# xflouris/libpll

Hardware: AMD Instinct MI355X
Metric: M CLV-site-updates/s (4x4 states x rates) (higher is better)
Workload: dtype f64

## Files before the change

### include/pll_amd.h

```cpp
#ifndef PLL_AMD_H_
#define PLL_AMD_H_

#include <stddef.h>
#include <stdint.h>
#include <stdio.h>

#ifdef __cplusplus
extern "C" {
#endif

#define PLL_EXPORT __attribute__((visibility("default")))


#define PLL_FAILURE 0
#define PLL_SUCCESS 1
#define PLL_FALSE 0
#define PLL_TRUE 1

#define PLL_ASCII_SIZE 256

#define PLL_SCALE_FACTOR 0x1p+256
#define PLL_SCALE_THRESHOLD 0x1p-256
#define PLL_SCALE_BUFFER_NONE (-1)
#define PLL_SCALE_RATE_MAXDIFF 4
// ... 885 lines not shown
PLL_EXPORT int pll_amd_set_deferral(pll_partition_t * partition, int on);
PLL_EXPORT int pll_amd_set_unstored_pairs(pll_partition_t * partition, int on);
PLL_EXPORT int pll_amd_unstored_stats(pll_partition_t * partition, unsigned long long * stats4);
PLL_EXPORT int pll_amd_set_pair_fold(pll_partition_t * partition, int on);
PLL_EXPORT int pll_amd_pair_fold_stats(pll_partition_t * partition, unsigned long long * stats4);
PLL_EXPORT int pll_amd_set_pair_row_capacity(pll_partition_t * partition, unsigned int rows);
PLL_EXPORT int pll_amd_pair_row_stats(pll_partition_t * partition, unsigned long long * stats4);
PLL_EXPORT int pll_amd_set_quad_rows(pll_partition_t * partition, int on, unsigned int min_sites_per_class);
PLL_EXPORT int pll_amd_set_quad_row_capacity(pll_partition_t * partition, unsigned int rows);
PLL_EXPORT int pll_amd_quad_row_stats(pll_partition_t * partition, unsigned long long * stats5);
PLL_EXPORT int pll_amd_quad_list_stats(pll_partition_t * partition, unsigned long long * stats3);
PLL_EXPORT int pll_amd_set_unstored_quad_products(pll_partition_t * partition, int on);
PLL_EXPORT int pll_amd_quad_product_stats(pll_partition_t * partition, unsigned long long * stats4);
PLL_EXPORT int pll_amd_set_quad_fold(pll_partition_t * partition, int on);
PLL_EXPORT int pll_amd_quad_fold_stats(pll_partition_t * partition, unsigned long long * stats4);
PLL_EXPORT int pll_amd_set_edge_fold(pll_partition_t * partition, int on);
PLL_EXPORT int pll_amd_edge_fold_stats(pll_partition_t * partition, unsigned long long * stats4);
PLL_EXPORT void * pll_amd_dev_clv(pll_partition_t * partition, unsigned int clv_index);

PLL_EXPORT int pll_amd_write_ceiling(pll_partition_t * partition, const pll_operation_t * operations, unsigned int count,
                                     unsigned int reps, float * ms_per_pass, double * bytes_per_pass);
PLL_EXPORT int pll_amd_list_kinds(pll_partition_t * partition, unsigned int * kinds8);
PLL_EXPORT int pll_amd_placement_info(pll_partition_t * partition, double * gbs, unsigned int cap, int * kept);
PLL_EXPORT int pll_amd_arena_fill_bandwidth(pll_partition_t * partition, double * gbs);

#ifdef __cplusplus
}
#endif
#endif
```

### include/pllhip.h

```cpp
#ifndef PLLHIP_H_
#define PLLHIP_H_

#include <stddef.h>
#include <stdint.h>

#ifdef __cplusplus
extern "C" {
#endif

#define PLLHIP_EXPORT __attribute__((visibility("default")))

typedef struct pllhip_ctx pllhip_ctx_t;

typedef struct pllhip_shape
{
  int device;
  unsigned int states;
  unsigned int rate_cats;
  unsigned int sites;
  unsigned int tips;
  unsigned int clv_buffers;
  unsigned int rate_matrices;
  unsigned int prob_matrices;
  unsigned int scale_buffers;
// ... 141 lines not shown
                                                      unsigned int lane);
PLLHIP_EXPORT int pllhip_fused_plan_dry_quads(unsigned int tips, unsigned int clv_buffers, unsigned int scale_buffers,
                                              int pattern_tip, unsigned int rate_cats, int rate_scalers, const pllhip_op_t * ops,
                                              unsigned int count, unsigned int nslots, const unsigned char * pinned,
                                              const int * edge4, unsigned int sites, int quads_on,
                                              unsigned int min_sites_per_class, const unsigned int * classes,
                                              const double * bounds, unsigned int * nkept, unsigned int * order_out,
                                              unsigned char * folded_out, int * ops_out, int * quads_out,
                                              unsigned int * counts_out);
PLLHIP_EXPORT int pllhip_fused_quad_rule_dry(int cherries, int instance, unsigned int n, unsigned int sites,
                                             unsigned int min_sites_per_class, int scales, double bound);
PLLHIP_EXPORT int pllhip_set_unstored_quad_products(pllhip_ctx_t * ctx, int on);
PLLHIP_EXPORT int pllhip_quad_product_stats(pllhip_ctx_t * ctx, unsigned long long * out4);
PLLHIP_EXPORT int pllhip_set_quad_fold(pllhip_ctx_t * ctx, int on);
PLLHIP_EXPORT int pllhip_quad_fold_stats(pllhip_ctx_t * ctx, unsigned long long * out4);
PLLHIP_EXPORT int pllhip_fused_plan_dry_quad_fold(unsigned int tips, unsigned int clv_buffers, unsigned int scale_buffers,
                                                  int pattern_tip, unsigned int rate_cats, int rate_scalers,
                                                  const pllhip_op_t * ops, unsigned int count, unsigned int nslots,
                                                  const unsigned char * pinned, const int * edge4, unsigned int sites,
                                                  int quads_on, unsigned int min_sites_per_class,
                                                  const unsigned int * classes, const double * bounds, int fold_on,
                                                  unsigned int * nkept, unsigned int * order_out, unsigned char * folded_out,
                                                  int * ops_out, int * quads_out, unsigned int * counts_out,
                                                  unsigned char * products_out, unsigned int * bytes_out,
                                                  unsigned char * qfolded_out, unsigned int * walked_out);
PLLHIP_EXPORT int pllhip_fused_plan_dry_quad_products(unsigned int tips, unsigned int clv_buffers, unsigned int scale_buffers,
                                                      int pattern_tip, unsigned int rate_cats, int rate_scalers,
                                                      const pllhip_op_t * ops, unsigned int count, unsigned int nslots,
                                                      const unsigned char * pinned, const int * edge4, unsigned int sites,
                                                      int quads_on, unsigned int min_sites_per_class,
// ... 305 lines not shown
```

### libpll_amd/csrc/hip/ctx.hip

```cpp
#include <dlfcn.h>
#include <sched.h>
#include <time.h>
#include <stdarg.h>
#include <stdlib.h>
#include <string.h>

#include <rccl/rccl.h>

#include <algorithm>
#include <string>
#include <vector>

#include <atomic>
#include "ctx.hpp"
#include "numerics.hpp"

static thread_local char g_err[512] = "";

void pllhip_set_error(const char * fmt, ...)
{
  va_list ap;
  va_start(ap, fmt);
  vsnprintf(g_err, sizeof(g_err), fmt, ap);
  va_end(ap);
// ... 298 lines not shown
    auto up = [](size_t b) { return (b + 4095) & ~(size_t)4095; };
    char * base = nullptr;
    if ((rc = alloc_arena_placed(c, &base, up(clv_b) + up(tip_b) + up(sc_b), shape->pattern_tip ? 0 : shape->tips,
                                 shape->clv_buffers, c->clv_stride * sizeof(double)))) goto fail;
    c->clv_arena = reinterpret_cast<double *>(base);
    if (tip_b) c->tipchars = reinterpret_cast<unsigned char *>(base + up(clv_b));
    c->scaler_arena = reinterpret_cast<unsigned int *>(base + up(clv_b) + up(tip_b));
    c->clv_arena_alloc_bytes = clv_b;
  }
  c->clv_arena_bytes = n_clv * c->clv_elems * sizeof(double);
  c->clv.assign(nodes, nullptr);
  for (unsigned int i = first; i < nodes; ++i)
    c->clv[i] = c->clv_arena + (size_t)(i - first) * c->clv_stride;
  if ((rc = dev_alloc(&c->pmatrix, (size_t)shape->prob_matrices * c->pmat_elems, true,
                      c->stream))) goto fail;
  if ((rc = dev_alloc(&c->eigenvals, (size_t)shape->rate_matrices * S, true, c->stream))) goto fail;
  if ((rc = dev_alloc(&c->eigenvecs, (size_t)shape->rate_matrices * S * S, true, c->stream))) goto fail;
  if ((rc = dev_alloc(&c->inv_eigenvecs, (size_t)shape->rate_matrices * S * S, true, c->stream))) goto fail;
  if ((rc = dev_alloc(&c->freqs, (size_t)shape->rate_matrices * S, true, c->stream))) goto fail;
  if ((rc = dev_alloc(&c->prop_invar, (size_t)shape->rate_matrices, true, c->stream))) goto fail;
  c->h_prop_invar.assign(shape->rate_matrices, 0.0);
  if ((rc = dev_alloc(&c->rates, R, true, c->stream))) goto fail;
  if ((rc = dev_alloc(&c->rate_weights, R, true, c->stream))) goto fail;
  if ((rc = dev_alloc(&c->pattern_weights, N + PLLHIP_TAIL_SITES, true, c->stream))) goto fail;
  if ((rc = dev_alloc(&c->tipmap, (size_t)256, true, c->stream))) goto fail;
  if ((rc = dev_alloc(&c->block_partials, (size_t)PLLHIP_REDUCE_BLOCKS * 2, true, c->stream))) goto fail;
  if ((rc = dev_alloc(&c->d_result, (size_t)4, true, c->stream))) goto fail;
  if ((rc = dev_alloc(&c->d_zero, (size_t)64, true, c->stream))) goto fail;
  HIP_TRY(hipHostMalloc((void **)&c->h_result, 4 * sizeof(double), hipHostMallocMapped));
  HIP_TRY(hipHostGetDevicePointer((void **)&c->h_result_dev, c->h_result, 0));
// ... 378 lines not shown
  if (!rc && freqs) rc = h2d(c, c->freqs + pi * S, freqs, S * sizeof(double));
  if (!rc) rc = h2d(c, c->prop_invar + pi, &prop_invar, sizeof(double));
  c->h_prop_invar[pi] = prop_invar;
  c->any_prop_invar = false;
  for (double p : c->h_prop_invar)
    if (p > 0) c->any_prop_invar = true;
  return rc;
}

extern "C" int pllhip_put_pmatrix(pllhip_ctx_t * c, unsigned int idx, const double * h)
{
  pllhip_edge_terms_drop(c);
  PLLHIP_ALL_SHARDS(c, pllhip_put_pmatrix(s, idx, h));
  PLLHIP_CERT_FIRST(c);
  if (idx >= c->sh.prob_matrices) { pllhip_set_error("pllhip_put_pmatrix: index %u", idx); return -1; }
  if (idx < c->pmat_min_entry.size() && c->pmat_min_entry[idx] != 0.0)
  {
    c->pmat_min_entry[idx] = c->pmat_min_rowsum[idx] = 0.0;
    ++c->layout_epoch;
  }
  return h2d(c, pllhip_pmat_ptr(c, idx), h, c->pmat_elems * sizeof(double));
}

extern "C" int pllhip_put_scaler(pllhip_ctx_t * c, unsigned int idx, const unsigned int * h)
{
  pllhip_edge_terms_drop(c);
  PLLHIP_ALL_SHARDS(c, pllhip_put_scaler(s, idx, h + lo * (c->sh.rate_scalers ? c->sh.rate_cats : 1)));
  PLLHIP_CERT_FIRST(c);
  if (idx >= c->sh.scale_buffers) { pllhip_set_error("pllhip_put_scaler: index %u", idx); return -1; }
  PLLHIP_DEFERRED_NEED(c, ~0u, ~0u, idx, -1);
// ... 376 lines not shown
```

### libpll_amd/csrc/hip/ctx.hpp

```cpp
#pragma once

#include <hip/hip_runtime.h>
#include <stdint.h>
#include <stdio.h>
#include <string.h>
#include <utility>
#include <vector>

#include "pllhip.h"

#define PLLHIP_MAX_RATE_CATS 64
#define PLLHIP_REDUCE_BLOCKS 65536
#define PLLHIP_HOSTSUM_MAX 8192

struct ncclComm;

struct pllhip_rep_work;

struct BatchScratch
{
  void * p = nullptr;
  size_t bytes = 0;
};
enum
// ... 16 lines not shown
  UNSTORED_NONE,
  UNSTORED_CHERRY,
  UNSTORED_PAIR,
  UNSTORED_FOLDED,
  UNSTORED_QUAD,
  UNSTORED_QUAD_FOLDED,
  UNSTORED_KINDS
};

struct pllhip_replicates
{
  pllhip_ctx * ctx;
  void * d_weights;
  size_t pitch;
  unsigned int count, width;
};

struct pllhip_ctx
{
  pllhip_shape_t sh;
  hipStream_t stream = nullptr;

  std::vector<pllhip_ctx *> shards;
  std::vector<size_t> shard_lo;
  bool shard_threads = true, shard_poll = true;
  bool shard_pin = false;
  struct pllhip_shard_pool * pool = nullptr;
  bool defer = false;
  unsigned long long pending_seq = 0;
  bool pending_hostsum = false, pending_spin = false, pending_stream_work = false;
// ... 74 lines not shown
    unsigned int * h_counts = nullptr;
    std::vector<quad_row> rows;
    unsigned int want = 0;
    unsigned int nstale = 0;
    unsigned long long clock = 0;
    unsigned long long stats[5] = {0, 0, 0, 0, 0};
  } quad_rows;
  bool quad_rows_on = true;
  unsigned int quad_min_sites_per_class = 64;
  std::vector<double> pmat_min_entry, pmat_min_rowsum;
  std::vector<double> h_eigenvals, h_eigenvecs, h_inv_eigenvecs, h_rates;
  std::vector<unsigned int> fused_last_quad_mats;
  unsigned int fused_last_quads_refused_by_bound = 0;
  unsigned int fused_last_quad_jobs = 0;
  unsigned long long quad_list_stats[3] = {0, 0, 0};
  struct deferred_clv
  {
    unsigned char kind = UNSTORED_NONE;
    unsigned int clv = 0;
    int scaler = -1;
    struct { unsigned int tip1 = 0, tip2 = 0; } cherry;
    struct { unsigned int rows[4] = {0, 0, 0, 0}; } pair;
    struct
    {
      unsigned int row[2] = {0, 0};
      unsigned int tips[2][4] = {{0, 0, 0, 0}, {0, 0, 0, 0}};
      unsigned int slot = 0;
    } quad;
    bool live() const { return kind != UNSTORED_NONE; }
    bool is_pair() const { return kind == UNSTORED_PAIR || kind == UNSTORED_FOLDED; }
// ... 233 lines not shown
static inline unsigned int * pllhip_scaler_ptr(const pllhip_ctx * c, int idx)
{
  return idx < 0 ? nullptr : c->scaler_arena + (size_t)idx * c->scaler_stride;
}

static inline const unsigned char * pllhip_tip_ptr(const pllhip_ctx * c, unsigned int tip)
{
  return c->tipchars + (size_t)tip * c->tip_stride;
}

static inline double * pllhip_pmat_ptr(const pllhip_ctx * c, unsigned int idx)
{
  return c->pmatrix + (size_t)idx * c->pmat_elems;
}

#define PLLHIP_INFINITY_CACHE_BYTES ((size_t)256 << 20)
static inline bool pllhip_use_nt(const pllhip_ctx * c)
{
  if (c->nt_override >= 0) return c->nt_override != 0;
  return c->clv_arena_bytes >= PLLHIP_INFINITY_CACHE_BYTES;
}

#define PLLHIP_STREAM_BLOCKS_PER_CU 256

static inline unsigned int pllhip_stream_grid(const pllhip_ctx * c, size_t items,
                                              unsigned int block)
{
  size_t need = (items + block - 1) / block;
  const size_t cap = (size_t)c->num_cus * PLLHIP_STREAM_BLOCKS_PER_CU;
  if (need < 1) need = 1;
// ... 135 lines not shown
```

### libpll_amd/csrc/hip/partials_fused.hip

```cpp
#include <algorithm>
#include <stdio.h>
#include <stdlib.h>
#include <type_traits>
#include <vector>

#include "ctx.hpp"
#include "numerics.hpp"
#include "partials_fused.hpp"

#define PLL_LDS __attribute__((address_space(3)))
#define PLL_GLOBAL __attribute__((address_space(1)))
typedef pll_v2d PLL_GLOBAL * global_v2d;
template <bool NT>
__device__ __forceinline__ void st16g(unsigned long long base, unsigned int byte_offset, double a, double b)
{
  const global_v2d p = (global_v2d)(base + byte_offset);
  const pll_v2d v = {a, b};
  if (NT) __builtin_nontemporal_store(v, p);
  else *p = v;
}

typedef const unsigned int __attribute__((address_space(4))) * const_words;
typedef const unsigned long long __attribute__((address_space(4))) * const_quads;
struct Rec
// ... 17 lines not shown
__device__ __forceinline__ unsigned int rec_req_rmat(const Rec & r) { return r.w[5]; }
__device__ __forceinline__ unsigned int rec_gather(const Rec & r) { return r.w[6]; }
__device__ __forceinline__ unsigned int rec_flags(const Rec & r) { return r.w[7]; }
__device__ __forceinline__ unsigned long long rec_parent(const Rec & r) { return rec_quad(r, 8); }
__device__ __forceinline__ unsigned long long rec_pscaler(const Rec & r) { return rec_quad(r, 10); }
__device__ __forceinline__ unsigned int rec_lslot(const Rec & r) { return r.w[12] & 0xffffu; }
__device__ __forceinline__ unsigned int rec_rslot(const Rec & r) { return r.w[12] >> 16; }
__device__ __forceinline__ unsigned int rec_pslot(const Rec & r) { return r.w[13] & 0xffffu; }
__device__ __forceinline__ unsigned int rec_src(const Rec & r) { return r.w[13] >> 16; }
__device__ __forceinline__ unsigned int rec_lcnt(const Rec & r) { return r.w[14] & 0xffffu; }
__device__ __forceinline__ unsigned int rec_rcnt(const Rec & r) { return r.w[14] >> 16; }
__device__ __forceinline__ unsigned int rec_pcnt(const Rec & r) { return r.w[15] & 0xffffu; }

constexpr unsigned int PLLHIP_QUAD_TABLE_WGS = 16;
template <int RC>
__global__ __launch_bounds__(256) void k_dna_quad_tables(const FusedPairJob * __restrict__ jobs, unsigned int njobs)
{
  const unsigned int i = blockIdx.x / PLLHIP_QUAD_TABLE_WGS, part = blockIdx.x % PLLHIP_QUAD_TABLE_WGS;
  if (i + 1 >= njobs || jobs[i].kind != 4) return;
  constexpr unsigned int ROW = RC * 4u, PER = 256u / ROW;
  const unsigned int ki = threadIdx.x % ROW, sub = threadIdx.x / ROW, rate4 = (ki >> 2) * 4u;
  const FusedPairJob & ja = jobs[i], & jb = jobs[i + 1];
  const PLL_GLOBAL double * pm = (const PLL_GLOBAL double *)ja.pmat;
  const PLL_GLOBAL unsigned short * patterns = (const PLL_GLOBAL unsigned short *)ja.kept;
  const unsigned int n = (unsigned int)ja.pad;
  const PLL_GLOBAL double * side_l[2] = {(const PLL_GLOBAL double *)ja.lmat, (const PLL_GLOBAL double *)jb.lmat};
  const PLL_GLOBAL double * side_r[2] = {(const PLL_GLOBAL double *)ja.rmat, (const PLL_GLOBAL double *)jb.rmat};
  const PLL_GLOBAL double * side_p[2] = {(const PLL_GLOBAL double *)jb.pmat, (const PLL_GLOBAL double *)jb.kept};
  const PLL_GLOBAL double * side_kept[2] = {(const PLL_GLOBAL double *)jb.copy, (const PLL_GLOBAL double *)jb.pad};
  double * tab = ja.tab;
  double * copy = ja.copy;
  double p[4], pf[2][4][4], l[2][4][4], r[2][4][4];
#pragma unroll
  for (int k = 0; k < 4; ++k) p[k] = pm[ki * 4u + k];
// ... 19 lines not shown
      double t[4];
#pragma unroll
      for (int k = 0; k < 4; ++k)
        t[k] = side_kept[s] ? side_kept[s][pair * ROW + rate4 + k] : masksum4(l[s][k], c1) * masksum4(r[s][k], c2);
#pragma unroll
      for (int k = 0; k < 4; ++k) f[s][k] = dot4(pf[s][k], t[0], t[1], t[2], t[3]);
    }
    const double q = dot4(p, f[0][0] * f[1][0], f[0][1] * f[1][1], f[0][2] * f[1][2], f[0][3] * f[1][3]);
    tab[cls * ROW + ki] = q;
    if (copy) copy[cls * ROW + ki] = q;
  }
}

template <int RC>
__global__ __launch_bounds__(256) void k_dna_pair_tables(const FusedPairJob * __restrict__ jobs, unsigned int njobs,
                                                         unsigned int * __restrict__ tile_counters)
{
  const unsigned int i = blockIdx.x >> 2, quarter = blockIdx.x & 3u;
  if (blockIdx.x == 0 && tile_counters) tile_counters[threadIdx.x * 32u] = 0u;
  if (i >= njobs) return;
  if (jobs[i].kind >= 4) return;
  if (jobs[i].kind >= 2)
  {
    constexpr unsigned int ROW = RC * 4u, PER = 256u / ROW, ROUNDS = 64u / PER;
    const unsigned int ki = threadIdx.x % ROW, sub = threadIdx.x / ROW, rate4 = (ki >> 2) * 4u;
    const PLL_GLOBAL double * pm = (const PLL_GLOBAL double *)jobs[i].pmat;
    double * tab = jobs[i].tab;
    double * copy = jobs[i].copy;
    double p[4];
#pragma unroll
    for (int k = 0; k < 4; ++k) p[k] = pm[ki * 4u + k];
    if (jobs[i].kind == 2)
    {
      const PLL_GLOBAL double * lm = (const PLL_GLOBAL double *)jobs[i].lmat, * rm = (const PLL_GLOBAL double *)jobs[i].rmat;
      double l[4][4], r[4][4];
// ... 1008 lines not shown
  if (f.rsc_slot >= 0) e.flags |= PLLHIP_FUSED_RCNT;
  e.lslot_b = (unsigned short)(f.lslot * in.slot.tile_bytes);
  e.rslot_b = (unsigned short)(f.rslot * in.slot.tile_bytes);
  e.lcnt_b = (unsigned short)((f.lsc_slot > 0 ? f.lsc_slot : 0) * in.slot.count_bytes);
  e.rcnt_b = (unsigned short)((f.rsc_slot > 0 ? f.rsc_slot : 0) * in.slot.count_bytes);
}

static void fused_encode(const FusedEncodeIn & in, const std::vector<std::vector<FusedOp>> & plans, const FusedAdmitted & adm,
                         const std::vector<FusedPairJob> * keep_jobs, const FusedEdge * edge, FusedEncoded & out)
{
  out.longest = adm.longest;
  for (size_t sg = 0; sg < plans.size(); ++sg) fused_encode_segment(in, plans[sg], adm.segs[sg], edge, out);
  if (keep_jobs) out.jobs.insert(out.jobs.end(), keep_jobs->begin(), keep_jobs->end());
}

static int fused_upload(pllhip_ctx * c, const FusedEncoded & enc)
{
  const size_t rec_bytes = enc.recs.size() * sizeof(FusedRec);
  const size_t seg_bytes = (size_t)PLLHIP_FUSED_MAX_SEGS * sizeof(FusedSeg);
  const size_t src_bytes = (enc.srcs.size() + 1) * sizeof(FusedSrc);
  const size_t job_bytes = (enc.jobs.size() + 1) * sizeof(FusedPairJob);
  const size_t tab_bytes = enc.rowtab.size() * sizeof(unsigned long long);
  const size_t segs_at = rec_bytes, srcs_at = segs_at + seg_bytes, jobs_at = srcs_at + src_bytes, rowtab_at = jobs_at + job_bytes;
  const size_t bytes = rowtab_at + tab_bytes;
  if (c->plan_cap < bytes)
  {
    HIP_TRY(hipStreamSynchronize(c->stream));
    for (int b = 0; b < 2; ++b)
    {
      if (c->h_plan[b]) HIP_TRY(hipHostFree(c->h_plan[b]));
// ... 13 lines not shown
  if (c->plan_pending[b]) HIP_TRY(hipEventSynchronize(c->plan_done[b]));
  char * stage = static_cast<char *>(c->h_plan[b]);
  memcpy(stage, enc.recs.data(), rec_bytes);
  memcpy(stage + segs_at, enc.segs.data(), enc.segs.size() * sizeof(FusedSeg));
  if (!enc.srcs.empty()) memcpy(stage + srcs_at, enc.srcs.data(), enc.srcs.size() * sizeof(FusedSrc));
  if (!enc.jobs.empty()) memcpy(stage + jobs_at, enc.jobs.data(), enc.jobs.size() * sizeof(FusedPairJob));
  memcpy(stage + rowtab_at, enc.rowtab.data(), tab_bytes);
  HIP_TRY(hipMemcpyAsync(c->d_plan, c->h_plan[b], bytes, hipMemcpyHostToDevice, c->stream));
  HIP_TRY(hipEventRecord(c->plan_done[b], c->stream));
  c->plan_pending[b] = true;
  c->fused_last_segs_offset = segs_at;
  c->fused_last_srcs_offset = srcs_at;
  c->fused_last_jobs_offset = jobs_at;
  c->fused_last_rowtab_offset = rowtab_at;
  c->fused_last_jobs = (unsigned int)enc.jobs.size();
  c->fused_last_quad_jobs = 0;
  for (const FusedPairJob & j : enc.jobs) c->fused_last_quad_jobs += j.kind == 4;
  c->quad_list_stats[0] = c->quad_list_stats[1] = c->fused_last_quad_jobs;
  c->quad_list_stats[2] += c->fused_last_quad_jobs;
  c->fused_last_longest = enc.longest;
  c->fused_last_nsegs = (unsigned int)enc.segs.size();
  c->fused_last_mode = enc.mode;
  c->fused_last_epoch = c->layout_epoch;
  return 0;
}

static int fused_device_buffers(pllhip_ctx * c, size_t pairtab_elems, bool edge)
{
  if (edge && !c->d_edge_terms)
    HIP_TRY(hipMalloc((void **)&c->d_edge_terms, ((size_t)c->sh.sites + PLLHIP_TAIL_SITES) * sizeof(double)));
  if (c->pairtab_elems < pairtab_elems)
  {
    HIP_TRY(hipStreamSynchronize(c->stream));
    if (c->d_pairtab) HIP_TRY(hipFree(c->d_pairtab));
    c->d_pairtab = nullptr;
    HIP_TRY(hipMalloc((void **)&c->d_pairtab, pairtab_elems * sizeof(double)));
    c->pairtab_elems = pairtab_elems;
    ++c->layout_epoch;
  }
  if (!c->fused_zero_row)
  {
    const size_t bytes = (size_t)c->sh.sites + PLLHIP_TAIL_SITES + 256;
    HIP_TRY(hipMalloc((void **)&c->fused_zero_row, bytes));
    HIP_TRY(hipMemsetAsync(c->fused_zero_row, 0, bytes, c->stream));
  }
  if (!c->d_sink) HIP_TRY(hipMalloc(&c->d_sink, (size_t)c->num_cus * 16 * PLLHIP_FUSED_SINK_GRANULES * sizeof(double2)));
  if (!c->d_tile_counter)
  {
    HIP_TRY(hipMalloc((void **)&c->d_tile_counter, 2 * PLLHIP_TILE_COUNTER_BYTES));
    HIP_TRY(hipMemsetAsync(c->d_tile_counter, 0, 2 * PLLHIP_TILE_COUNTER_BYTES, c->stream));
  }
  return 0;
}
// ... 243 lines not shown
}

int pllhip_relaunch_fused(pllhip_ctx * c)
{
  const unsigned int count = c->fused_last_count, nslots = c->fused_last_nslots, njobs = c->fused_last_jobs;
  const int mode = c->fused_last_mode;
  static_assert(PLLHIP_TILE_COUNTER_BYTES == 256 * 128, "one counter per thread of k_dna_pair_tables' first workgroup");
  if (const int rc = pllhip_pair_rows_refresh(c)) return rc;
  const FusedRec * d_plan = (const FusedRec *)c->d_plan;
  const FusedPairJob * d_jobs = (const FusedPairJob *)(static_cast<const char *>(c->d_plan) + c->fused_last_jobs_offset);
  const FusedBases bases = {c->pmatrix, c->d_pairtab,
                            (const unsigned long long *)(static_cast<const char *>(c->d_plan) + c->fused_last_rowtab_offset),
                            (const FusedSrc *)(static_cast<const char *>(c->d_plan) + c->fused_last_srcs_offset),
                            (const FusedSeg *)(static_cast<const char *>(c->d_plan) + c->fused_last_segs_offset),
                            c->fused_last_nsegs};
  if (njobs)
  {
    switch (c->sh.rate_cats)
    {
      case 1: k_dna_pair_tables<1><<<4 * njobs, 256, 0, c->stream>>>(d_jobs, njobs, nullptr); break;
      case 2: k_dna_pair_tables<2><<<4 * njobs, 256, 0, c->stream>>>(d_jobs, njobs, nullptr); break;
      case 8: k_dna_pair_tables<8><<<4 * njobs, 256, 0, c->stream>>>(d_jobs, njobs, nullptr); break;
      default: k_dna_pair_tables<4><<<4 * njobs, 256, 0, c->stream>>>(d_jobs, njobs, nullptr); break;
    }
    HIP_TRY(hipGetLastError());
  }
  if (c->fused_last_quad_jobs)
  {
    const unsigned int nwg = PLLHIP_QUAD_TABLE_WGS * njobs;
    switch (c->sh.rate_cats)
    {
      case 1: k_dna_quad_tables<1><<<nwg, 256, 0, c->stream>>>(d_jobs, njobs); break;
      case 2: k_dna_quad_tables<2><<<nwg, 256, 0, c->stream>>>(d_jobs, njobs); break;
      case 4: k_dna_quad_tables<4><<<nwg, 256, 0, c->stream>>>(d_jobs, njobs); break;
      default: pllhip_set_error("quad tables: %u categories", c->sh.rate_cats); return -1;
    }
    HIP_TRY(hipGetLastError());
  }
  switch (c->sh.rate_cats)
  {
    case 1: return launch_fused_rc<1>(c, d_plan, bases, count, nslots, mode, c->fused_last_edge);
    case 2: return launch_fused_rc<2>(c, d_plan, bases, count, nslots, mode, c->fused_last_edge);
    case 8: return launch_fused_rc<8>(c, d_plan, bases, count, nslots, mode, c->fused_last_edge);
    default: return launch_fused_rc<4>(c, d_plan, bases, count, nslots, mode, c->fused_last_edge);
  }
}


extern "C" unsigned long long pllhip_fused_group_mask_dry(unsigned int gw, unsigned long long mask)
{
  switch (gw)
  {
    case 2: return pllhip_fused_group_mask<2>(mask);
    case 4: return pllhip_fused_group_mask<4>(mask);
    case 8: return pllhip_fused_group_mask<8>(mask);
    case 16: return pllhip_fused_group_mask<16>(mask);
    default: return 0;
  }
}

// ... 64 lines not shown
```

### libpll_amd/csrc/hip/partials_fused.hpp

```cpp
#ifndef PLLHIP_PARTIALS_FUSED_HPP_
#define PLLHIP_PARTIALS_FUSED_HPP_

#include <utility>
#include <vector>

#include "ctx.hpp"

constexpr int PLLHIP_FUSED_J = 2;

struct FusedSlotSize
{
  unsigned int count_words, tile_bytes, count_bytes;
  unsigned int bytes() const { return tile_bytes + count_bytes; }
};
inline FusedSlotSize pllhip_fused_slot_size(unsigned int rate_cats, bool rate_scalers)
{
  const unsigned int sps = 64 / (2 * rate_cats);
  const unsigned int cw = rate_scalers ? 32 : (sps < 4 ? 4 : sps);
  return {cw, PLLHIP_FUSED_J * 64u * 16u, PLLHIP_FUSED_J * cw * 4u};
}

enum { FUSED_G_NONE = 0, FUSED_G_TIP = 1, FUSED_G_PAIR = 2, FUSED_G_CHERRY_NEW = 3, FUSED_G_CHERRY_KEPT = 4 };
struct FusedOperand
{
// ... 470 lines not shown
  const pllhip_op_t * ops = nullptr;
  unsigned int count = 0;
  const FusedEdge * edge = nullptr;
  const unsigned char * pinned = nullptr;
  std::vector<pllhip_ctx::deferred_clv> left;
  bool fold = false;
  const PartialsArgs * args = nullptr;
  const int * kinds = nullptr;
  const FusedExtra * extras = nullptr;
  const unsigned int * rows8 = nullptr;
  unsigned int max_segments = 1;
  const FusedDeferral * dd = nullptr;
  FusedQuadFold folded;
  unsigned int nfolded = 0;
};
int pllhip_launch_fused(pllhip_ctx * c, const std::vector<std::vector<FusedOp>> & plans, unsigned int nslots,
                        const std::vector<FusedPairJob> * keep_jobs = nullptr, const FusedEdge * edge = nullptr,
                        FusedQuadProducts * quad_products = nullptr);
int pllhip_relaunch_fused(pllhip_ctx * c);

#endif
```

### libpll_amd/csrc/hip/pmatrix.hip

```cpp
#include <algorithm>
#include <math.h>

#include "ctx.hpp"
#include "numerics.hpp"
#include "pmatrix_entry.hpp"

#define PMAT_INLINE 256

struct PmatArgs
{
  double * pmatrix;
  const double * eigenvals;
  const double * eigenvecs;
  const double * inv_eigenvecs;
  const double * prop_invar;
  const double * rates;
  const unsigned int * matrix_indices;
  const double * branch_lengths;
  unsigned int states, rate_cats;
  unsigned int split;
  unsigned int params_indices[PLLHIP_MAX_RATE_CATS];
  unsigned int mi_inline[PMAT_INLINE];
  double bl_inline[PMAT_INLINE];
};
// ... 146 lines not shown
    c->pmat_min_rowsum[mi] = rs;
  }
  if (changed) ++c->layout_epoch;
}

extern "C" int pllhip_update_pmatrices(pllhip_ctx_t * c, const unsigned int * h_params_indices,
                                       const unsigned int * h_matrix_indices,
                                       const double * h_branch_lengths, unsigned int count)
{
  pllhip_edge_terms_drop(c);
  PLLHIP_ALL_SHARDS_PAR(c, pllhip_update_pmatrices(s, h_params_indices, h_matrix_indices, h_branch_lengths, count));
  if (!count) return 0;
  HIP_TRY(hipSetDevice(c->sh.device));
  PLLHIP_CERT_FIRST(c);
  pllhip_pmat_bounds_update(c, h_params_indices, h_matrix_indices, h_branch_lengths, count);
  return pllhip_pmatrices_to(c, c->pmatrix, c->sh.prob_matrices, h_params_indices, h_matrix_indices, h_branch_lengths,
                             count);
}
```

### libpll_amd/csrc/host/partition.c

```c
#include <stdarg.h>
#include <stdio.h>

#include "internal.h"

__thread int pll_errno;
__thread char pll_errmsg[200] = {0};

int pll_amd_mirror_mode = 0;
static __thread int g_device = -1;
static int g_device_default = -1;

void pll_amd_set_error(int code, const char * fmt, ...)
{
  va_list ap;
  pll_errno = code;
  va_start(ap, fmt);
  vsnprintf(pll_errmsg, sizeof(pll_errmsg), fmt, ap);
  va_end(ap);
}

int pll_amd_fail_hip(int rc, const char * what)
{
  pll_amd_set_error(PLL_ERROR_HIP_RUNTIME, "%s: %s (rc=%d)", what, pllhip_last_error(), rc);
  return PLL_FAILURE;
// ... 830 lines not shown

int pll_amd_quad_fold_stats(pll_partition_t * p, unsigned long long * stats4)
{
  int rc = pllhip_quad_fold_stats(pll_amd_priv(p)->ctx, stats4);
  if (rc) return pll_amd_fail_hip(rc, "quad fold stats");
  return PLL_SUCCESS;
}

int pll_amd_set_quad_fold(pll_partition_t * p, int on)
{
  int rc = pllhip_set_quad_fold(pll_amd_priv(p)->ctx, on);
  if (rc) return pll_amd_fail_hip(rc, "set quad fold");
  return PLL_SUCCESS;
}

int pll_amd_pair_fold_stats(pll_partition_t * p, unsigned long long * stats4)
{
  int rc = pllhip_pair_fold_stats(pll_amd_priv(p)->ctx, stats4);
  if (rc) return pll_amd_fail_hip(rc, "pair fold stats");
  return PLL_SUCCESS;
}

int pll_amd_set_pair_fold(pll_partition_t * p, int on)
{
  int rc = pllhip_set_pair_fold(pll_amd_priv(p)->ctx, on);
  if (rc) return pll_amd_fail_hip(rc, "set pair fold");
  return PLL_SUCCESS;
}

int pll_amd_set_pair_row_capacity(pll_partition_t * p, unsigned int rows)
// ... 96 lines not shown
```

### libpll_amd/pllapi.py

```python
import ctypes as C
import os

import numpy as np

SCALE_BUFFER_NONE = -1
ATTRIB_ARCH_CPU = 0
ERROR_PARAM_INVALID = 113
ATTRIB_ARCH_SSE = 1 << 0
ATTRIB_ARCH_AVX = 1 << 1
ATTRIB_ARCH_AVX2 = 1 << 2
ATTRIB_PATTERN_TIP = 1 << 4
ATTRIB_AB_LEWIS = 1 << 5
ATTRIB_AB_FELSENSTEIN = 2 << 5
ATTRIB_AB_STAMATAKIS = 3 << 5
ATTRIB_AB_FLAG = 1 << 8
ATTRIB_RATE_SCALERS = 1 << 9
ATTRIB_SITE_REPEATS = 1 << 10
GAMMA_RATES_MEAN = 0
GAMMA_RATES_MEDIAN = 1


class PartitionStruct(C.Structure):
    _fields_ = [
        ("tips", C.c_uint), ("clv_buffers", C.c_uint), ("states", C.c_uint),
# ... 248 lines not shown
                lib.pll_amd_pair_fold_stats.argtypes = [_PP, C.POINTER(C.c_ulonglong)]
            if hasattr(lib, "pll_amd_set_pair_row_capacity"):
                lib.pll_amd_set_pair_row_capacity.argtypes = [_PP, C.c_uint]
                lib.pll_amd_pair_row_stats.argtypes = [_PP, C.POINTER(C.c_ulonglong)]
            if hasattr(lib, "pll_amd_set_quad_rows"):
                lib.pll_amd_set_quad_rows.argtypes = [_PP, C.c_int, C.c_uint]
                lib.pll_amd_set_quad_row_capacity.argtypes = [_PP, C.c_uint]
                lib.pll_amd_quad_row_stats.argtypes = [_PP, C.POINTER(C.c_ulonglong)]
                lib.pll_amd_quad_list_stats.argtypes = [_PP, C.POINTER(C.c_ulonglong)]
            if hasattr(lib, "pll_amd_set_unstored_quad_products"):
                lib.pll_amd_set_unstored_quad_products.argtypes = [_PP, C.c_int]
                lib.pll_amd_quad_product_stats.argtypes = [_PP, C.POINTER(C.c_ulonglong)]
            if hasattr(lib, "pll_amd_set_quad_fold"):
                lib.pll_amd_set_quad_fold.argtypes = [_PP, C.c_int]
                lib.pll_amd_quad_fold_stats.argtypes = [_PP, C.POINTER(C.c_ulonglong)]
            if hasattr(lib, "pll_amd_set_edge_fold"):
                lib.pll_amd_set_edge_fold.argtypes = [_PP, C.c_int]
                lib.pll_amd_edge_fold_stats.argtypes = [_PP, C.POINTER(C.c_ulonglong)]
                lib.pll_amd_push_clv.argtypes = [_PP, C.c_uint]
                lib.pll_amd_push_scaler.argtypes = [_PP, C.c_uint]
            if hasattr(lib, "pll_amd_write_ceiling"):
                lib.pll_amd_write_ceiling.argtypes = [_PP, C.c_void_p, C.c_uint, C.c_uint, C.POINTER(C.c_float),
                                                      C.POINTER(C.c_double)]
                lib.pll_amd_list_kinds.argtypes = [_PP, _up]
            lib.pll_amd_eigen_decompose.argtypes = [C.c_uint, _dp, _dp, _dp, _dp, _dp]
            if hasattr(lib, "pll_amd_insertion_loglikelihood"):
                lib.pll_amd_insertion_loglikelihood.argtypes = [_PP, C.c_void_p, C.c_uint, _up, C.c_void_p, _dp,
                                                                C.c_uint, _up, _dp]
            if hasattr(lib, "pll_amd_optimize_branch_lengths"):
                lib.pll_amd_optimize_branch_lengths.argtypes = [_PP, C.c_void_p, C.c_uint, _up, C.c_double,
# ... 1051 lines not shown
        self._check(self.lib.pll_amd_set_unstored_quad_products(self.ptr, 1 if on else 0), "pll_amd_set_unstored_quad_products")

    def quad_product_stats(self):
        buf = (C.c_ulonglong * 4)()
        self._check(self.lib.pll_amd_quad_product_stats(self.ptr, buf), "pll_amd_quad_product_stats")
        return dict(zip(("live", "ops_unstored", "launches", "materialised"), (int(v) for v in buf)))

    def set_quad_fold(self, on):
        self._check(self.lib.pll_amd_set_quad_fold(self.ptr, 1 if on else 0), "pll_amd_set_quad_fold")

    def quad_fold_stats(self):
        buf = (C.c_ulonglong * 4)()
        self._check(self.lib.pll_amd_quad_fold_stats(self.ptr, buf), "pll_amd_quad_fold_stats")
        return dict(zip(("live", "ops_folded", "plans", "materialised"), (int(v) for v in buf)))

    def unstored_stats(self):
        buf = (C.c_ulonglong * 4)()
        self._check(self.lib.pll_amd_unstored_stats(self.ptr, buf), "pll_amd_unstored_stats")
        return dict(zip(("unstored_now", "ops_unstored", "launches", "materialised"), (int(v) for v in buf)))

    def set_edge_fold(self, on):
        self._check(self.lib.pll_amd_set_edge_fold(self.ptr, 1 if on else 0), "pll_amd_set_edge_fold")

    def edge_fold_stats(self):
        buf = (C.c_ulonglong * 4)()
        self._check(self.lib.pll_amd_edge_fold_stats(self.ptr, buf), "pll_amd_edge_fold_stats")
        return [int(v) for v in buf]

    def dev_clv(self, idx):
        return self.lib.pll_amd_dev_clv(self.ptr, idx)
# ... 37 lines not shown
```

Baseline: 220,600.

## Skip rebuilding fused pair/quad tables whose probability matrices are unchanged

Adds a write clock to every probability matrix and records which matrices each fused pair or quad table job reads. Before launching the table-building kernels, the host computes a stale mask and launches only when some job's inputs changed since the last build; kernels skip jobs that are not stale. This aims to cut redundant table construction across repeated CLV passes with unchanged branch lengths. The cost is host-side bookkeeping, a 128-byte mask kernel argument, and correctness now depends on every pmatrix write path calling the stamp hook.

```diff
diff --git a/include/pll_amd.h b/include/pll_amd.h
--- a/include/pll_amd.h
+++ b/include/pll_amd.h
@@ -923,6 +923,10 @@
 PLL_EXPORT int pll_amd_quad_product_stats(pll_partition_t * partition, unsigned long long * stats4);
 PLL_EXPORT int pll_amd_set_quad_fold(pll_partition_t * partition, int on);
 PLL_EXPORT int pll_amd_quad_fold_stats(pll_partition_t * partition, unsigned long long * stats4);
+PLL_EXPORT int pll_amd_set_table_reuse(pll_partition_t * partition, int on);
+PLL_EXPORT int pll_amd_table_reuse_stats(pll_partition_t * partition, unsigned long long * stats4);
+PLL_EXPORT int pll_amd_table_jobs(pll_partition_t * partition, unsigned int * kinds, unsigned int * mats,
+                                  unsigned int cap, unsigned int * njobs);
 PLL_EXPORT int pll_amd_set_edge_fold(pll_partition_t * partition, int on);
 PLL_EXPORT int pll_amd_edge_fold_stats(pll_partition_t * partition, unsigned long long * stats4);
 PLL_EXPORT void * pll_amd_dev_clv(pll_partition_t * partition, unsigned int clv_index);
diff --git a/include/pllhip.h b/include/pllhip.h
--- a/include/pllhip.h
+++ b/include/pllhip.h
@@ -179,6 +179,15 @@
 PLLHIP_EXPORT int pllhip_quad_product_stats(pllhip_ctx_t * ctx, unsigned long long * out4);
 PLLHIP_EXPORT int pllhip_set_quad_fold(pllhip_ctx_t * ctx, int on);
 PLLHIP_EXPORT int pllhip_quad_fold_stats(pllhip_ctx_t * ctx, unsigned long long * out4);
+PLLHIP_EXPORT int pllhip_set_table_reuse(pllhip_ctx_t * ctx, int on);
+PLLHIP_EXPORT int pllhip_table_reuse_stats(pllhip_ctx_t * ctx, unsigned long long * out4);
+PLLHIP_EXPORT int pllhip_table_jobs(pllhip_ctx_t * ctx, unsigned int * kinds, unsigned int * mats, unsigned int cap,
+                                    unsigned int * njobs);
+PLLHIP_EXPORT int pllhip_table_reuse_dry(const unsigned int * kinds, const unsigned int * mats, unsigned int njobs,
+                                         const unsigned long long * written, unsigned int nmats, unsigned long long built,
+                                         int all, unsigned long long * mask_out, unsigned int * out4);
+PLLHIP_EXPORT int pllhip_pmat_stamp_dry(unsigned long long * written, unsigned int nmats, unsigned long long * clock,
+                                        unsigned int idx);
 PLLHIP_EXPORT int pllhip_fused_plan_dry_quad_fold(unsigned int tips, unsigned int clv_buffers, unsigned int scale_buffers,
                                                   int pattern_tip, unsigned int rate_cats, int rate_scalers,
                                                   const pllhip_op_t * ops, unsigned int count, unsigned int nslots,
diff --git a/libpll_amd/csrc/hip/ctx.hip b/libpll_amd/csrc/hip/ctx.hip
--- a/libpll_amd/csrc/hip/ctx.hip
+++ b/libpll_amd/csrc/hip/ctx.hip
@@ -336,6 +336,7 @@
     c->clv[i] = c->clv_arena + (size_t)(i - first) * c->clv_stride;
   if ((rc = dev_alloc(&c->pmatrix, (size_t)shape->prob_matrices * c->pmat_elems, true,
                       c->stream))) goto fail;
+  c->pmat_written.assign(shape->prob_matrices, 0ull);
   if ((rc = dev_alloc(&c->eigenvals, (size_t)shape->rate_matrices * S, true, c->stream))) goto fail;
   if ((rc = dev_alloc(&c->eigenvecs, (size_t)shape->rate_matrices * S * S, true, c->stream))) goto fail;
   if ((rc = dev_alloc(&c->inv_eigenvecs, (size_t)shape->rate_matrices * S * S, true, c->stream))) goto fail;
@@ -744,6 +745,7 @@
   PLLHIP_ALL_SHARDS(c, pllhip_put_pmatrix(s, idx, h));
   PLLHIP_CERT_FIRST(c);
   if (idx >= c->sh.prob_matrices) { pllhip_set_error("pllhip_put_pmatrix: index %u", idx); return -1; }
+  pllhip_pmat_stamp(c, idx);
   if (idx < c->pmat_min_entry.size() && c->pmat_min_entry[idx] != 0.0)
   {
     c->pmat_min_entry[idx] = c->pmat_min_rowsum[idx] = 0.0;
diff --git a/libpll_amd/csrc/hip/ctx.hpp b/libpll_amd/csrc/hip/ctx.hpp
--- a/libpll_amd/csrc/hip/ctx.hpp
+++ b/libpll_amd/csrc/hip/ctx.hpp
@@ -54,6 +54,15 @@
   void * d_weights;
   size_t pitch;
   unsigned int count, width;
+};
+
+#define PLLHIP_JOB_MATS 7
+#define PLLHIP_JOB_MAT_NONE 0xffffffffu
+#define PLLHIP_JOB_MAT_UNKNOWN 0xfffffffeu
+struct FusedJobReads
+{
+  unsigned int kind;
+  unsigned int mat[PLLHIP_JOB_MATS];
 };
 
 struct pllhip_ctx
@@ -158,6 +167,13 @@
   unsigned int fused_last_quads_refused_by_bound = 0;
   unsigned int fused_last_quad_jobs = 0;
   unsigned long long quad_list_stats[3] = {0, 0, 0};
+  unsigned long long pmat_clock = 0;
+  std::vector<unsigned long long> pmat_written;
+  std::vector<FusedJobReads> fused_last_job_reads;
+  unsigned long long fused_tables_clock = 0;
+  bool fused_tables_all_stale = true;
+  bool table_reuse = true;
+  unsigned long long table_reuse_stats[4] = {0, 0, 0, 0};
   struct deferred_clv
   {
     unsigned char kind = UNSTORED_NONE;
@@ -421,6 +437,16 @@
   return c->pmatrix + (size_t)idx * c->pmat_elems;
 }
 
+static inline void pllhip_pmat_stamp_at(unsigned long long * written, unsigned int nmats, unsigned long long * clock, unsigned int idx)
+{
+  if (idx < nmats) written[idx] = ++*clock;
+}
+static inline void pllhip_pmat_stamp(pllhip_ctx * c, unsigned int idx)
+{
+  pllhip_pmat_stamp_at(c->pmat_written.data(), (unsigned int)c->pmat_written.size(), &c->pmat_clock, idx);
+}
+static inline void pllhip_tables_mark_stale(pllhip_ctx * c) { c->fused_tables_all_stale = true; }
+
 #define PLLHIP_INFINITY_CACHE_BYTES ((size_t)256 << 20)
 static inline bool pllhip_use_nt(const pllhip_ctx * c)
 {
diff --git a/libpll_amd/csrc/hip/partials_fused.hip b/libpll_amd/csrc/hip/partials_fused.hip
--- a/libpll_amd/csrc/hip/partials_fused.hip
+++ b/libpll_amd/csrc/hip/partials_fused.hip
@@ -55,10 +55,11 @@
 
 constexpr unsigned int PLLHIP_QUAD_TABLE_WGS = 16;
 template <int RC>
-__global__ __launch_bounds__(256) void k_dna_quad_tables(const FusedPairJob * __restrict__ jobs, unsigned int njobs)
+__global__ __launch_bounds__(256) void k_dna_quad_tables(const FusedPairJob * __restrict__ jobs, unsigned int njobs,
+                                                         const FusedStaleMask stale)
 {
   const unsigned int i = blockIdx.x / PLLHIP_QUAD_TABLE_WGS, part = blockIdx.x % PLLHIP_QUAD_TABLE_WGS;
-  if (i + 1 >= njobs || jobs[i].kind != 4) return;
+  if (i + 1 >= njobs || !pllhip_fused_job_runs(stale, i) || jobs[i].kind != 4) return;
   constexpr unsigned int ROW = RC * 4u, PER = 256u / ROW;
   const unsigned int ki = threadIdx.x % ROW, sub = threadIdx.x / ROW, rate4 = (ki >> 2) * 4u;
   const FusedPairJob & ja = jobs[i], & jb = jobs[i + 1];
@@ -108,11 +109,12 @@
 
 template <int RC>
 __global__ __launch_bounds__(256) void k_dna_pair_tables(const FusedPairJob * __restrict__ jobs, unsigned int njobs,
-                                                         unsigned int * __restrict__ tile_counters)
+                                                         unsigned int * __restrict__ tile_counters, const FusedStaleMask stale)
 {
   const unsigned int i = blockIdx.x >> 2, quarter = blockIdx.x & 3u;
   if (blockIdx.x == 0 && tile_counters) tile_counters[threadIdx.x * 32u] = 0u;
   if (i >= njobs) return;
+  if (!pllhip_fused_job_runs(stale, i)) return;
   if (jobs[i].kind >= 4) return;
   if (jobs[i].kind >= 2)
   {
@@ -1151,6 +1153,38 @@
   if (keep_jobs) out.jobs.insert(out.jobs.end(), keep_jobs->begin(), keep_jobs->end());
 }
 
+static void fused_job_reads(const pllhip_ctx * c, const std::vector<FusedPairJob> & jobs, std::vector<FusedJobReads> & out)
+{
+  auto index_of = [&](const double * m) {
+    if (!m) return PLLHIP_JOB_MAT_NONE;
+    const size_t idx = m >= c->pmatrix ? (size_t)(m - c->pmatrix) / c->pmat_elems : ~(size_t)0;
+    return idx < c->sh.prob_matrices ? (unsigned int)idx : PLLHIP_JOB_MAT_UNKNOWN;
+  };
+  out.assign(jobs.size(), FusedJobReads());
+  for (size_t i = 0; i < jobs.size(); ++i)
+  {
+    const FusedPairJob & j = jobs[i];
+    FusedJobReads & r = out[i];
+    r.kind = (unsigned int)j.kind;
+    for (unsigned int & m : r.mat) m = PLLHIP_JOB_MAT_NONE;
+    if (j.kind == 5ull) continue;
+    if (j.kind == 4ull)
+    {
+      if (i + 1 >= jobs.size()) continue;
+      const FusedPairJob & b = jobs[i + 1];
+      if (!b.copy) { r.mat[0] = index_of(j.lmat); r.mat[1] = index_of(j.rmat); }
+      if (!b.pad) { r.mat[2] = index_of(b.lmat); r.mat[3] = index_of(b.rmat); }
+      r.mat[4] = index_of(b.pmat);
+      r.mat[5] = index_of(b.kept);
+      r.mat[6] = index_of(j.pmat);
+      continue;
+    }
+    if (j.kind != 3ull) r.mat[0] = index_of(j.lmat);
+    if (j.kind == 1ull || j.kind == 2ull) r.mat[1] = index_of(j.rmat);
+    if (j.kind >= 2ull) r.mat[2] = index_of(j.pmat);
+  }
+}
+
 static int fused_upload(pllhip_ctx * c, const FusedEncoded & enc)
 {
   const size_t rec_bytes = enc.recs.size() * sizeof(FusedRec);
@@ -1194,6 +1228,8 @@
   c->fused_last_jobs_offset = jobs_at;
   c->fused_last_rowtab_offset = rowtab_at;
   c->fused_last_jobs = (unsigned int)enc.jobs.size();
+  fused_job_reads(c, enc.jobs, c->fused_last_job_reads);
+  pllhip_tables_mark_stale(c);
   c->fused_last_quad_jobs = 0;
   for (const FusedPairJob & j : enc.jobs) c->fused_last_quad_jobs += j.kind == 4;
   c->quad_list_stats[0] = c->quad_list_stats[1] = c->fused_last_quad_jobs;
@@ -1217,6 +1253,7 @@
     HIP_TRY(hipMalloc((void **)&c->d_pairtab, pairtab_elems * sizeof(double)));
     c->pairtab_elems = pairtab_elems;
     ++c->layout_epoch;
+    pllhip_tables_mark_stale(c);
   }
   if (!c->fused_zero_row)
   {
@@ -1490,29 +1527,41 @@
                             (const FusedSrc *)(static_cast<const char *>(c->d_plan) + c->fused_last_srcs_offset),
                             (const FusedSeg *)(static_cast<const char *>(c->d_plan) + c->fused_last_segs_offset),
                             c->fused_last_nsegs};
-  if (njobs)
+  FusedStaleMask stale;
+  unsigned int runs[4];
+  pllhip_fused_stale_jobs(c->fused_last_job_reads.data(), njobs, c->pmat_written.data(), (unsigned int)c->pmat_written.size(),
+                          c->fused_tables_clock, c->fused_tables_all_stale || !c->table_reuse, stale, runs);
+  pllhip_tables_mark_stale(c);
+  if (runs[2])
   {
     switch (c->sh.rate_cats)
     {
-      case 1: k_dna_pair_tables<1><<<4 * njobs, 256, 0, c->stream>>>(d_jobs, njobs, nullptr); break;
-      case 2: k_dna_pair_tables<2><<<4 * njobs, 256, 0, c->stream>>>(d_jobs, njobs, nullptr); break;
-      case 8: k_dna_pair_tables<8><<<4 * njobs, 256, 0, c->stream>>>(d_jobs, njobs, nullptr); break;
-      default: k_dna_pair_tables<4><<<4 * njobs, 256, 0, c->stream>>>(d_jobs, njobs, nullptr); break;
+      case 1: k_dna_pair_tables<1><<<4 * njobs, 256, 0, c->stream>>>(d_jobs, njobs, nullptr, stale); break;
+      case 2: k_dna_pair_tables<2><<<4 * njobs, 256, 0, c->stream>>>(d_jobs, njobs, nullptr, stale); break;
+      case 8: k_dna_pair_tables<8><<<4 * njobs, 256, 0, c->stream>>>(d_jobs, njobs, nullptr, stale); break;
+      default: k_dna_pair_tables<4><<<4 * njobs, 256, 0, c->stream>>>(d_jobs, njobs, nullptr, stale); break;
     }
     HIP_TRY(hipGetLastError());
   }
-  if (c->fused_last_quad_jobs)
+  if (runs[3])
   {
     const unsigned int nwg = PLLHIP_QUAD_TABLE_WGS * njobs;
     switch (c->sh.rate_cats)
     {
-      case 1: k_dna_quad_tables<1><<<nwg, 256, 0, c->stream>>>(d_jobs, njobs); break;
-      case 2: k_dna_quad_tables<2><<<nwg, 256, 0, c->stream>>>(d_jobs, njobs); break;
-      case 4: k_dna_quad_tables<4><<<nwg, 256, 0, c->stream>>>(d_jobs, njobs); break;
+      case 1: k_dna_quad_tables<1><<<nwg, 256, 0, c->stream>>>(d_jobs, njobs, stale); break;
+      case 2: k_dna_quad_tables<2><<<nwg, 256, 0, c->stream>>>(d_jobs, njobs, stale); break;
+      case 4: k_dna_quad_tables<4><<<nwg, 256, 0, c->stream>>>(d_jobs, njobs, stale); break;
       default: pllhip_set_error("quad tables: %u categories", c->sh.rate_cats); return -1;
     }
     HIP_TRY(hipGetLastError());
   }
+  c->fused_tables_all_stale = false;
+  c->fused_tables_clock = c->pmat_clock;
+  const unsigned int would = (njobs > c->fused_last_quad_jobs * 2u ? 1u : 0u) + (c->fused_last_quad_jobs ? 1u : 0u);
+  c->table_reuse_stats[0] += runs[0];
+  c->table_reuse_stats[1] += runs[1];
+  c->table_reuse_stats[2] += runs[2] + runs[3];
+  c->table_reuse_stats[3] += would - (runs[2] + runs[3]);
   switch (c->sh.rate_cats)
   {
     case 1: return launch_fused_rc<1>(c, d_plan, bases, count, nslots, mode, c->fused_last_edge);
@@ -1520,6 +1569,73 @@
     case 8: return launch_fused_rc<8>(c, d_plan, bases, count, nslots, mode, c->fused_last_edge);
     default: return launch_fused_rc<4>(c, d_plan, bases, count, nslots, mode, c->fused_last_edge);
   }
+}
+
+extern "C" int pllhip_set_table_reuse(pllhip_ctx_t * c, int on)
+{
+  pllhip_edge_terms_drop(c);
+  PLLHIP_ALL_SHARDS(c, pllhip_set_table_reuse(s, on));
+  c->table_reuse = on != 0;
+  pllhip_tables_mark_stale(c);
+  return 0;
+}
+
+extern "C" int pllhip_table_reuse_stats(pllhip_ctx_t * c, unsigned long long * out4)
+{
+  for (int t = 0; t < 4; ++t) out4[t] = 0;
+  auto add = [&](const pllhip_ctx * s) {
+    for (int t = 0; t < 4; ++t) out4[t] += s->table_reuse_stats[t];
+  };
+  if (c->shards.empty()) add(c);
+  for (const pllhip_ctx * s : c->shards) add(s);
+  return 0;
+}
+
+extern "C" int pllhip_table_jobs(pllhip_ctx_t * c, unsigned int * kinds, unsigned int * mats, unsigned int cap, unsigned int * njobs)
+{
+  if (!njobs) return -1;
+  const pllhip_ctx * s = c->shards.empty() ? c : c->shards[0];
+  const unsigned int n = s->fused_last_ops.empty() ? 0u : (unsigned int)s->fused_last_job_reads.size();
+  *njobs = n;
+  for (unsigned int i = 0; i < n && i < cap && kinds && mats; ++i)
+  {
+    kinds[i] = s->fused_last_job_reads[i].kind;
+    memcpy(mats + (size_t)i * PLLHIP_JOB_MATS, s->fused_last_job_reads[i].mat, sizeof(s->fused_last_job_reads[i].mat));
+  }
+  return 0;
+}
+
+extern "C" int pllhip_table_reuse_dry(const unsigned int * kinds, const unsigned int * mats, unsigned int njobs,
+                                      const unsigned long long * written, unsigned int nmats, unsigned long long built,
+                                      int all, unsigned long long * mask_out, unsigned int * out4)
+{
+  if (!out4 || !mask_out || (njobs && (!kinds || !mats)) || (nmats && !written)) return 1;
+  std::vector<FusedJobReads> jobs(njobs);
+  for (unsigned int i = 0; i < njobs; ++i)
+  {
+    if (kinds[i] > 5u || (kinds[i] == 5u && (i == 0 || kinds[i - 1] != 4u)) || (kinds[i] == 4u && (i + 1 >= njobs || kinds[i + 1] != 5u)))
+      return 1;
+    jobs[i].kind = kinds[i];
+    for (unsigned int k = 0; k < PLLHIP_JOB_MATS; ++k)
+    {
+      const unsigned int m = mats[(size_t)i * PLLHIP_JOB_MATS + k];
+      if (m >= nmats && m != PLLHIP_JOB_MAT_NONE && m != PLLHIP_JOB_MAT_UNKNOWN) return 1;
+      jobs[i].mat[k] = m;
+    }
+  }
+  FusedStaleMask mask;
+  pllhip_fused_stale_jobs(jobs.data(), njobs, written, nmats, built, all != 0, mask, out4);
+  for (unsigned int w = 0; w < PLLHIP_TABLE_MASK_WORDS; ++w) mask_out[w] = 0ull;
+  for (unsigned int i = 0; i < PLLHIP_TABLE_MASK_JOBS; ++i)
+    if (pllhip_fused_job_runs(mask, i)) mask_out[i >> 6] |= 1ull << (i & 63u);
+  return 0;
+}
+
+extern "C" int pllhip_pmat_stamp_dry(unsigned long long * written, unsigned int nmats, unsigned long long * clock, unsigned int idx)
+{
+  if (!written || !clock || idx >= nmats) return 1;
+  pllhip_pmat_stamp_at(written, nmats, clock, idx);
+  return 0;
 }
 
 
diff --git a/libpll_amd/csrc/hip/partials_fused.hpp b/libpll_amd/csrc/hip/partials_fused.hpp
--- a/libpll_amd/csrc/hip/partials_fused.hpp
+++ b/libpll_amd/csrc/hip/partials_fused.hpp
@@ -508,6 +508,43 @@
   FusedQuadFold folded;
   unsigned int nfolded = 0;
 };
+constexpr unsigned int PLLHIP_TABLE_MASK_WORDS = 16u, PLLHIP_TABLE_MASK_JOBS = 64u * PLLHIP_TABLE_MASK_WORDS;
+struct FusedStaleMask
+{
+  unsigned long long w[PLLHIP_TABLE_MASK_WORDS];
+};
+inline void pllhip_fused_stale_jobs(const FusedJobReads * jobs, unsigned int njobs, const unsigned long long * written,
+                                    unsigned int nmats, unsigned long long built, bool all, FusedStaleMask & mask,
+                                    unsigned int * out4)
+{
+  auto is_stale = [&](const FusedJobReads & j) {
+    for (unsigned int m : j.mat)
+      if (m != PLLHIP_JOB_MAT_NONE && (m >= nmats || written[m] > built)) return true;
+    return false;
+  };
+  bool any = false;
+  for (unsigned int i = 0; i < njobs && !any; ++i) any = jobs[i].kind != 5u && is_stale(jobs[i]);
+  if (any && njobs > PLLHIP_TABLE_MASK_JOBS) all = true;
+  memset(&mask, 0, sizeof(mask));
+  out4[0] = out4[1] = out4[2] = out4[3] = 0u;
+  for (unsigned int i = 0; i < njobs; ++i)
+  {
+    if (jobs[i].kind == 5u) continue;
+    if (!all && !is_stale(jobs[i]))
+    {
+      ++out4[1];
+      continue;
+    }
+    ++out4[0];
+    out4[jobs[i].kind == 4u ? 3 : 2] = 1u;
+    if (i < PLLHIP_TABLE_MASK_JOBS) mask.w[i >> 6] |= 1ull << (i & 63u);
+  }
+}
+__host__ __device__ __forceinline__ bool pllhip_fused_job_runs(const FusedStaleMask & mask, unsigned int i)
+{
+  return i >= PLLHIP_TABLE_MASK_JOBS || ((mask.w[i >> 6] >> (i & 63u)) & 1ull) != 0ull;
+}
+
 int pllhip_launch_fused(pllhip_ctx * c, const std::vector<std::vector<FusedOp>> & plans, unsigned int nslots,
                         const std::vector<FusedPairJob> * keep_jobs = nullptr, const FusedEdge * edge = nullptr,
                         FusedQuadProducts * quad_products = nullptr);
diff --git a/libpll_amd/csrc/hip/pmatrix.hip b/libpll_amd/csrc/hip/pmatrix.hip
--- a/libpll_amd/csrc/hip/pmatrix.hip
+++ b/libpll_amd/csrc/hip/pmatrix.hip
@@ -184,6 +184,7 @@
   HIP_TRY(hipSetDevice(c->sh.device));
   PLLHIP_CERT_FIRST(c);
   pllhip_pmat_bounds_update(c, h_params_indices, h_matrix_indices, h_branch_lengths, count);
+  for (unsigned int i = 0; i < count; ++i) pllhip_pmat_stamp(c, h_matrix_indices[i]);
   return pllhip_pmatrices_to(c, c->pmatrix, c->sh.prob_matrices, h_params_indices, h_matrix_indices, h_branch_lengths,
                              count);
 }
diff --git a/libpll_amd/csrc/host/partition.c b/libpll_amd/csrc/host/partition.c
--- a/libpll_amd/csrc/host/partition.c
+++ b/libpll_amd/csrc/host/partition.c
@@ -868,6 +868,27 @@
   return PLL_SUCCESS;
 }
 
+int pll_amd_table_reuse_stats(pll_partition_t * p, unsigned long long * stats4)
+{
+  int rc = pllhip_table_reuse_stats(pll_amd_priv(p)->ctx, stats4);
+  if (rc) return pll_amd_fail_hip(rc, "table reuse stats");
+  return PLL_SUCCESS;
+}
+
+int pll_amd_table_jobs(pll_partition_t * p, unsigned int * kinds, unsigned int * mats, unsigned int cap, unsigned int * njobs)
+{
+  int rc = pllhip_table_jobs(pll_amd_priv(p)->ctx, kinds, mats, cap, njobs);
+  if (rc) return pll_amd_fail_hip(rc, "table jobs");
+  return PLL_SUCCESS;
+}
+
+int pll_amd_set_table_reuse(pll_partition_t * p, int on)
+{
+  int rc = pllhip_set_table_reuse(pll_amd_priv(p)->ctx, on);
+  if (rc) return pll_amd_fail_hip(rc, "set table reuse");
+  return PLL_SUCCESS;
+}
+
 int pll_amd_pair_fold_stats(pll_partition_t * p, unsigned long long * stats4)
 {
   int rc = pllhip_pair_fold_stats(pll_amd_priv(p)->ctx, stats4);
diff --git a/libpll_amd/pllapi.py b/libpll_amd/pllapi.py
--- a/libpll_amd/pllapi.py
+++ b/libpll_amd/pllapi.py
@@ -286,6 +286,10 @@
             if hasattr(lib, "pll_amd_set_quad_fold"):
                 lib.pll_amd_set_quad_fold.argtypes = [_PP, C.c_int]
                 lib.pll_amd_quad_fold_stats.argtypes = [_PP, C.POINTER(C.c_ulonglong)]
+            if hasattr(lib, "pll_amd_set_table_reuse"):
+                lib.pll_amd_set_table_reuse.argtypes = [_PP, C.c_int]
+                lib.pll_amd_table_reuse_stats.argtypes = [_PP, C.POINTER(C.c_ulonglong)]
+                lib.pll_amd_table_jobs.argtypes = [_PP, _up, _up, C.c_uint, _up]
             if hasattr(lib, "pll_amd_set_edge_fold"):
                 lib.pll_amd_set_edge_fold.argtypes = [_PP, C.c_int]
                 lib.pll_amd_edge_fold_stats.argtypes = [_PP, C.POINTER(C.c_ulonglong)]
@@ -1367,6 +1371,22 @@
         self._check(self.lib.pll_amd_quad_fold_stats(self.ptr, buf), "pll_amd_quad_fold_stats")
         return dict(zip(("live", "ops_folded", "plans", "materialised"), (int(v) for v in buf)))
 
+    def set_table_reuse(self, on):
+        self._check(self.lib.pll_amd_set_table_reuse(self.ptr, 1 if on else 0), "pll_amd_set_table_reuse")
+
+    def table_reuse_stats(self):
+        buf = (C.c_ulonglong * 4)()
+        self._check(self.lib.pll_amd_table_reuse_stats(self.ptr, buf), "pll_amd_table_reuse_stats")
+        return dict(zip(("jobs_run", "jobs_skipped", "launches", "launches_skipped"), (int(v) for v in buf)))
+
+    def table_jobs(self):
+        n = C.c_uint(0)
+        self._check(self.lib.pll_amd_table_jobs(self.ptr, None, None, 0, C.byref(n)), "pll_amd_table_jobs")
+        kinds, mats = np.zeros(n.value, dtype=np.uint32), np.zeros((n.value, 7), dtype=np.uint32)
+        self._check(self.lib.pll_amd_table_jobs(self.ptr, kinds.ctypes.data_as(_up), mats.ctypes.data_as(_up), n.value, C.byref(n)),
+                    "pll_amd_table_jobs")
+        return kinds, mats
+
     def unstored_stats(self):
         buf = (C.c_ulonglong * 4)()
         self._check(self.lib.pll_amd_unstored_stats(self.ptr, buf), "pll_amd_unstored_stats")
```

New measurement: 229,700, median of 6. 4.1% higher.
